# Tariq-Abuhashim/semantic-slam

Hardware: AMD Instinct MI355X
Metric: Mvoxels/sec integrated, 512³ grid @ 640×480 depth; achieved HBM GB/s %peak (higher is better)
Workload: dtype f32

## Files before the change

### include/tsdf_hip_diag.h

```cpp
#ifndef TSDF_HIP_DIAG_H
#define TSDF_HIP_DIAG_H

#include "tsdf_hip.h"

#ifdef __cplusplus
extern "C" {
#endif


int tsdf_integrate_sequence_timed(tsdf_volume *vol, const float *depth_dev, const float *cam2world,
                                  int32_t n_frames, float *elapsed_ms);

int tsdf_integrate_frames_timed(tsdf_volume *vol, const float *const *depth_dev, const uint8_t *const *masks_dev,
                                const float *cam2world, int32_t n_frames, float *elapsed_ms);


int tsdf_probe_graph_replay(tsdf_volume *vol, const float *depth_dev, const float *cam2world, int32_t n_frames,
                            int32_t iters, float *ms_launches, float *ms_graph);

int tsdf_probe_stream(tsdf_volume *vol, int32_t non_temporal, int32_t n_iters, float *elapsed_ms);


int tsdf_selftest_fastdiv(int32_t device, uint64_t seed, uint64_t n_samples, float fx, float cx,
                          uint64_t *mismatches, float first_bad[4]);

int tsdf_selftest_fastdiv_band(int32_t device, uint64_t seed, uint64_t n_samples, uint64_t *mismatches,
                               float first_bad[4]);

int tsdf_selftest_round(int32_t device, uint64_t *mismatches, float first_bad[4]);

int tsdf_selftest_tile_tables(int32_t device, const float *depth_dev, const uint8_t *mask_dev, int32_t im_height,
                              int32_t im_width, float max_depth, uint64_t *mismatches);


int32_t tsdf_frames_per_launch(const tsdf_volume *vol);
int tsdf_shortcut_stats(tsdf_volume *vol, int32_t enable, uint64_t counts_out[3]);
int tsdf_brick_list_stats(tsdf_volume *vol, uint64_t counts_out[4]);
int tsdf_classification_info(tsdf_volume *vol, double info_out[2]);

int tsdf_summary_stats(tsdf_volume *vol, uint64_t out[3]);
int tsdf_summary_words(tsdf_volume *vol, uint32_t *out_host, int64_t capacity, int64_t *count);

int tsdf_store_stats(tsdf_volume *vol, int64_t out[9]);

int tsdf_last_cam2base(const tsdf_volume *vol, float out[16]);


int tsdf_set_kernel_variant(tsdf_volume *vol, int32_t variant);

int tsdf_set_brick_shape(tsdf_volume *vol, int32_t quads, int32_t rows, int32_t slices);
int tsdf_brick_shape(const tsdf_volume *vol, int32_t shape_out[3]);
int tsdf_default_brick_shape(const tsdf_config *cfg, int32_t shape_out[3]);

#ifdef __cplusplus
}
#endif
#endif
```

### semantic_slam_amd/capi.py

```python
import ctypes as C
import os

import numpy as np

_PKG = os.path.dirname(os.path.abspath(__file__))
LIB_PATH = os.environ.get("TSDF_HIP_LIB") or os.path.join(_PKG, "libtsdf_hip.so")

ABI_SYMBOLS = [
    "tsdf_config_default", "tsdf_create", "tsdf_destroy", "tsdf_reset", "tsdf_integrate",
    "tsdf_integrate_u16", "tsdf_convert_depth_u16", "tsdf_set_deferral",
    "tsdf_integrate_device", "tsdf_integrate_cam2base", "tsdf_integrate_masked_device",
    "tsdf_integrate_frames_device",
    "tsdf_sync", "tsdf_download", "tsdf_copy_slices", "tsdf_upload", "tsdf_refresh_summary", "tsdf_device_ptrs", "tsdf_slab_voxels", "tsdf_frames_per_launch", "tsdf_shortcut_stats", "tsdf_brick_list_stats", "tsdf_classification_info", "tsdf_store_stats", "tsdf_summary_stats", "tsdf_summary_words",
    "tsdf_get_config", "tsdf_last_cam2base", "tsdf_set_stream", "tsdf_get_stream",
    "tsdf_count_surface", "tsdf_extract_surface", "tsdf_extract_crossings", "tsdf_extract_mesh", "tsdf_save_mesh_ply", "tsdf_save_mesh_welded_ply", "tsdf_save_ply", "tsdf_save_bin", "tsdf_load_bin", "tsdf_save_state", "tsdf_load_state",
    "tsdf_integrate_sequence_timed", "tsdf_integrate_frames_timed", "tsdf_probe_graph_replay", "tsdf_probe_stream", "tsdf_selftest_fastdiv", "tsdf_selftest_fastdiv_band", "tsdf_selftest_round", "tsdf_selftest_tile_tables", "tsdf_set_kernel_variant", "tsdf_set_brick_shape", "tsdf_brick_shape", "tsdf_default_brick_shape", "tsdf_last_error",
    "tsdf_version", "tsdf_multiply_matrix", "tsdf_invert_matrix",
    "tsdf_labels_enable", "tsdf_compose_labels", "tsdf_integrate_labels_device", "tsdf_integrate_frames_labels_device",
    "tsdf_download_labels",
    "tsdf_colour_enable", "tsdf_integrate_colour_device", "tsdf_integrate_rgbd", "tsdf_download_colour",
    "tsdf_raycast_params_default", "tsdf_raycast_device", "tsdf_raycast", "tsdf_batch_raycast_device",
    "tsdf_track_params_default", "tsdf_track", "tsdf_track_system",
    "tsdf_batch_track", "tsdf_batch_track_system", "tsdf_track_member_systems",
    "tsdf_fuse_params_default", "tsdf_fuse_volume",
    "tsdf_extent_params_default", "tsdf_volume_extent", "tsdf_batch_extents", "tsdf_group_extent", "tsdf_extent_combine",
    "tsdf_extent_metric", "tsdf_extent_regrid",
    "tsdf_associate_params_default", "tsdf_associate_count", "tsdf_associate_assign", "tsdf_batch_associate",
    "tsdf_segment_params_default", "tsdf_segmenter_create", "tsdf_segmenter_destroy", "tsdf_segmenter_set_stream",
    "tsdf_segment_depth_device", "tsdf_segment_refine_masks_device", "tsdf_segment_frame",
    "tsdf_object_origin", "tsdf_batch_create", "tsdf_batch_destroy", "tsdf_batch_size", "tsdf_batch_volume",
    "tsdf_batch_integrate_device", "tsdf_batch_sync",
    "tsdf_group_create", "tsdf_group_destroy", "tsdf_group_size", "tsdf_group_voxels", "tsdf_group_volume",
    "tsdf_group_integrate", "tsdf_group_integrate_frames", "tsdf_group_set_deferral", "tsdf_group_sync", "tsdf_group_reset", "tsdf_group_download",
    "tsdf_group_extract_surface", "tsdf_group_extract_crossings", "tsdf_group_extract_mesh",
    "tsdf_group_save_ply", "tsdf_group_save_mesh_ply", "tsdf_group_save_bin",
]
DIAG_SYMBOLS = [
    "tsdf_integrate_sequence_timed", "tsdf_integrate_frames_timed",
    "tsdf_probe_graph_replay", "tsdf_probe_stream",
    "tsdf_selftest_fastdiv", "tsdf_selftest_fastdiv_band", "tsdf_selftest_round", "tsdf_selftest_tile_tables",
    "tsdf_shortcut_stats", "tsdf_brick_list_stats", "tsdf_classification_info", "tsdf_store_stats", "tsdf_summary_stats", "tsdf_summary_words", "tsdf_frames_per_launch", "tsdf_last_cam2base",
    "tsdf_set_kernel_variant", "tsdf_set_brick_shape", "tsdf_brick_shape", "tsdf_default_brick_shape",
]


class TsdfError(RuntimeError):
    pass


SHIPPED_VARIANTS = (0, 1, 3, 7, 8)


def experiments_build():
    return b"+experiments" in load().tsdf_version()


def variants(*wanted):
    exp = experiments_build()
    return [v for v in wanted if v in SHIPPED_VARIANTS or exp]


class TsdfConfig(C.Structure):
    _fields_ = [
        ("im_height", C.c_int32), ("im_width", C.c_int32),
# ... 106 lines not shown
    L.tsdf_destroy.argtypes = [vp]
    L.tsdf_reset.argtypes = [vp]
    L.tsdf_integrate.argtypes = [vp, vp, vp]
    L.tsdf_set_deferral.argtypes = [vp, C.c_int32]
    L.tsdf_integrate_u16.argtypes = [vp, vp, C.c_float, C.c_int32, C.c_int32, vp]
    L.tsdf_convert_depth_u16.argtypes = [vp, vp, vp, C.c_float, C.c_int32, C.c_int32]
    L.tsdf_integrate_device.argtypes = [vp, vp, vp]
    L.tsdf_integrate_cam2base.argtypes = [vp, vp, vp]
    L.tsdf_integrate_masked_device.argtypes = [vp, vp, vp, vp]
    L.tsdf_integrate_frames_device.argtypes = [vp, vp, vp, vp, C.c_int32]
    L.tsdf_sync.argtypes = [vp]
    L.tsdf_download.argtypes = [vp, vp, vp]
    L.tsdf_upload.argtypes = [vp, vp, vp]
    L.tsdf_copy_slices.argtypes = [vp, C.c_int32, C.c_int32, vp, vp]
    L.tsdf_refresh_summary.argtypes = [vp]
    L.tsdf_device_ptrs.argtypes = [vp, C.POINTER(vp), C.POINTER(vp)]
    L.tsdf_slab_voxels.argtypes = [vp]
    L.tsdf_slab_voxels.restype = C.c_int64
    L.tsdf_frames_per_launch.argtypes = [vp]
    L.tsdf_frames_per_launch.restype = C.c_int32
    L.tsdf_shortcut_stats.argtypes = [vp, C.c_int32, vp]
    L.tsdf_classification_info.argtypes = [vp, vp]
    L.tsdf_brick_list_stats.argtypes = [vp, vp]
    if hasattr(L, "tsdf_store_stats"):
        L.tsdf_store_stats.argtypes = [vp, i64p]
    if hasattr(L, "tsdf_summary_stats"):
        L.tsdf_summary_stats.argtypes = [vp, vp]
    if hasattr(L, "tsdf_summary_words"):
        L.tsdf_summary_words.argtypes = [vp, vp, C.c_int64, i64p]
    L.tsdf_get_config.argtypes = [vp, C.POINTER(TsdfConfig)]
    L.tsdf_last_cam2base.argtypes = [vp, vp]
    L.tsdf_set_stream.argtypes = [vp, vp]
    L.tsdf_get_stream.argtypes = [vp, C.POINTER(vp)]
    L.tsdf_count_surface.argtypes = [vp, C.c_float, i64p]
    L.tsdf_extract_surface.argtypes = [vp, C.c_float, vp, C.c_int64, i64p]
    L.tsdf_extract_crossings.argtypes = [vp, vp, vp, C.c_float, vp, C.c_int64, i64p]
    L.tsdf_extract_mesh.argtypes = [vp, vp, vp, C.c_float, vp, C.c_int64, i64p]
    L.tsdf_save_mesh_ply.argtypes = [vp, C.c_char_p, C.c_float]
    L.tsdf_save_mesh_welded_ply.argtypes = [vp, C.c_char_p, C.c_float]
    L.tsdf_save_ply.argtypes = [vp, C.c_char_p, C.c_float]
    L.tsdf_save_bin.argtypes = [vp, C.c_char_p]
    L.tsdf_load_bin.argtypes = [vp, C.c_char_p]
    L.tsdf_save_state.argtypes = [vp, C.c_char_p]
    L.tsdf_load_state.argtypes = [vp, C.c_char_p]
    L.tsdf_integrate_sequence_timed.argtypes = [vp, vp, vp, C.c_int32, f32p]
    L.tsdf_integrate_frames_timed.argtypes = [vp, vp, vp, vp, C.c_int32, f32p]
    L.tsdf_probe_graph_replay.argtypes = [vp, vp, vp, C.c_int32, C.c_int32, f32p, f32p]
    L.tsdf_probe_stream.argtypes = [vp, C.c_int32, C.c_int32, f32p]
    L.tsdf_selftest_fastdiv.argtypes = [C.c_int32, C.c_uint64, C.c_uint64, C.c_float, C.c_float, C.POINTER(C.c_uint64), f32p]
    L.tsdf_selftest_fastdiv_band.argtypes = [C.c_int32, C.c_uint64, C.c_uint64, C.POINTER(C.c_uint64), f32p]
    L.tsdf_selftest_round.argtypes = [C.c_int32, C.POINTER(C.c_uint64), f32p]
    L.tsdf_selftest_tile_tables.argtypes = [C.c_int32, vp, vp, C.c_int32, C.c_int32, C.c_float, C.POINTER(C.c_uint64)]
    L.tsdf_set_kernel_variant.argtypes = [vp, C.c_int32]
    L.tsdf_set_brick_shape.argtypes = [vp, C.c_int32, C.c_int32, C.c_int32]
    L.tsdf_brick_shape.argtypes = [vp, C.POINTER(C.c_int32)]
    L.tsdf_default_brick_shape.argtypes = [C.POINTER(TsdfConfig), C.POINTER(C.c_int32)]
    L.tsdf_last_error.restype = C.c_char_p
    L.tsdf_version.restype = C.c_char_p
    L.tsdf_multiply_matrix.argtypes = [vp, vp, vp]
    L.tsdf_multiply_matrix.restype = None
    L.tsdf_invert_matrix.argtypes = [vp, vp]
    L.tsdf_labels_enable.argtypes = [vp, C.c_float]
    L.tsdf_compose_labels.argtypes = [vp, vp, vp, vp, C.c_int32, vp, vp]
    L.tsdf_integrate_labels_device.argtypes = [vp, vp, vp, vp, vp]
    L.tsdf_download_labels.argtypes = [vp, vp, vp, vp]
    L.tsdf_integrate_frames_labels_device.argtypes = [vp, vp, vp, vp, vp, C.c_int32]
    L.tsdf_colour_enable.argtypes = [vp]
    L.tsdf_integrate_colour_device.argtypes = [vp, vp, vp, vp]
    L.tsdf_integrate_rgbd.argtypes = [vp, vp, vp, vp]
    L.tsdf_download_colour.argtypes = [vp, vp]
    L.tsdf_raycast_params_default.argtypes = [C.POINTER(TsdfConfig), C.POINTER(RaycastParams)]
    L.tsdf_raycast_device.argtypes = [vp, C.POINTER(RaycastParams), vp, vp, vp, vp, vp]
    L.tsdf_raycast.argtypes = [vp, C.POINTER(RaycastParams), vp, vp, vp, vp, vp]
# ... 101 lines not shown


def invert_matrix(m):
    out = np.zeros(16, np.float32)
    m = _f32(m, 16)
    ok = load().tsdf_invert_matrix(m.ctypes.data, out.ctypes.data)
    return bool(ok), out


def selftest_fastdiv(n_samples, seed=1, device=0, fx=535.4, cx=320.1):
    cnt = C.c_uint64()
    bad = (C.c_float * 4)()
    check(load().tsdf_selftest_fastdiv(device, seed, n_samples, fx, cx, C.byref(cnt), bad), "tsdf_selftest_fastdiv")
    return cnt.value, list(bad)


def selftest_fastdiv_band(n_samples, seed=1, device=0):
    cnt = C.c_uint64()
    bad = (C.c_float * 4)()
    check(load().tsdf_selftest_fastdiv_band(device, seed, n_samples, C.byref(cnt), bad), "tsdf_selftest_fastdiv_band")
    return cnt.value, list(bad)


def object_origin(depth_ptr, mask_ptr, h, w, K, device=0):
    k = _f32(K, 9)
    out = np.empty(3, np.float32)
    check(load().tsdf_object_origin(device, depth_ptr, mask_ptr, h, w, k.ctypes.data, out.ctypes.data), "tsdf_object_origin")
    return out


def raycast_params_default(cfg):
    p = RaycastParams()
    check(load().tsdf_raycast_params_default(C.byref(cfg), C.byref(p)), "tsdf_raycast_params_default")
    return p


def track_params_default(cfg):
    p = TrackParams()
    check(load().tsdf_track_params_default(C.byref(cfg), C.byref(p)), "tsdf_track_params_default")
    return p


def fuse_params_default(cfg):
    p = FuseParams()
    check(load().tsdf_fuse_params_default(C.byref(cfg), C.byref(p)), "tsdf_fuse_params_default")
    return p
# ... 172 lines not shown
        return self

    def __exit__(self, *exc):
        self.close()

    def __del__(self):
        try:
            self.close()
        except Exception:
            pass

    @property
    def n_voxels(self):
        return int(self.lib.tsdf_slab_voxels(self._h))

    def shortcut_stats(self, enable=True):
        out = (C.c_uint64 * 3)()
        check(self.lib.tsdf_shortcut_stats(self._h, 1 if enable else 0, out), "tsdf_shortcut_stats")
        return tuple(int(x) for x in out)

    def brick_list_stats(self):
        out = (C.c_uint64 * 4)()
        check(self.lib.tsdf_brick_list_stats(self._h, out), "tsdf_brick_list_stats")
        return tuple(int(x) for x in out)

    def classification_info(self):
        out = (C.c_double * 2)()
        check(self.lib.tsdf_classification_info(self._h, out), "tsdf_classification_info")
        return float(out[0]), int(out[1])

    def store_stats(self):
        out = (C.c_int64 * 9)()
        check(self.lib.tsdf_store_stats(self._h, out), "tsdf_store_stats")
        return {name: tuple(int(x) for x in out[3 * k:3 * k + 3]) for k, name in enumerate(("frames", "masks", "tables"))}

    def summary_stats(self):
        out = (C.c_uint64 * 3)()
        check(self.lib.tsdf_summary_stats(self._h, out), "tsdf_summary_stats")
        return tuple(int(x) for x in out)

    def summary_words(self):
        n = C.c_int64(0)
        check(self.lib.tsdf_summary_words(self._h, None, 0, C.byref(n)), "tsdf_summary_words")
        out = np.zeros(int(n.value), np.uint32)
        if out.size:
            check(self.lib.tsdf_summary_words(self._h, out.ctypes.data, out.size, C.byref(n)), "tsdf_summary_words")
# ... 516 lines not shown
```

### semantic_slam_amd/csrc/tsdf_diag.hip.h

```cpp
#pragma once

namespace {

template <typename Queue>
int time_on_stream(tsdf_volume *v, const char *who, float *elapsed_ms, Queue &&queue)
{
    Event e0, e1;
    HIP_TRY(event_create(e0, hipEventDefault));
    HIP_TRY(event_create(e1, hipEventDefault));
    HIP_TRY(hipEventRecord(e0, v->stream));
    const int rc = queue();
    hipError_t er = hipEventRecord(e1, v->stream);
    hipError_t es = hipEventSynchronize(e1);
    float ms = 0.f;
    hipError_t et = hipEventElapsedTime(&ms, e0, e1);
    if (rc) return rc;
    if (er != hipSuccess || es != hipSuccess || et != hipSuccess)
        return fail(TSDF_ERR_HIP, "%s: event timing failed", who);
    *elapsed_ms = ms;
    return TSDF_OK;
}

int frames_timed(tsdf_volume *v, const float *const *depth_dev, const uint8_t *const *masks_dev,
                 const float *cam2world, int32_t n_frames, float *elapsed_ms, const char *who)
// ... 108 lines not shown
    if (e == hipSuccess) e = hipMemcpy(first_bad, d_bad, 4 * sizeof(float), hipMemcpyDeviceToHost);
    if (e != hipSuccess) return fail(TSDF_ERR_HIP, "tsdf_selftest_fastdiv: %s", hipGetErrorString(e));
    *mismatches = cnt;
    return TSDF_OK;
}

int tsdf_selftest_fastdiv_band(int32_t device, uint64_t seed, uint64_t n_samples, uint64_t *mismatches, float first_bad[4])
{
    if (!mismatches || !first_bad) return fail(TSDF_ERR_INVALID, "tsdf_selftest_fastdiv_band: NULL argument");
    HIP_TRY(hipSetDevice(device));
    DevPtr<unsigned long long> d_cnt;
    DevPtr<float> d_bad;
    HIP_TRY(dev_alloc(d_cnt, sizeof(unsigned long long)));
    HIP_TRY(dev_alloc(d_bad, 4 * sizeof(float)));
    HIP_TRY(hipMemset(d_cnt, 0, sizeof(unsigned long long)));
    HIP_TRY(hipMemset(d_bad, 0, 4 * sizeof(float)));
    hipLaunchKernelGGL(tsdfk::selftest_fastdiv_band, dim3(256 * 8), dim3(256), 0, 0, seed, n_samples, d_cnt, d_bad);
    hipError_t e = hipGetLastError();
    if (e == hipSuccess) e = hipDeviceSynchronize();
    unsigned long long cnt = 0;
    if (e == hipSuccess) e = hipMemcpy(&cnt, d_cnt, sizeof cnt, hipMemcpyDeviceToHost);
    if (e == hipSuccess) e = hipMemcpy(first_bad, d_bad, 4 * sizeof(float), hipMemcpyDeviceToHost);
    if (e != hipSuccess) return fail(TSDF_ERR_HIP, "tsdf_selftest_fastdiv_band: %s", hipGetErrorString(e));
    *mismatches = cnt;
    return TSDF_OK;
}

int tsdf_selftest_round(int32_t device, uint64_t *mismatches, float first_bad[4])
{
    if (!mismatches || !first_bad) return fail(TSDF_ERR_INVALID, "tsdf_selftest_round: NULL argument");
    HIP_TRY(hipSetDevice(device));
    DevPtr<unsigned long long> d_cnt;
    DevPtr<float> d_bad;
    HIP_TRY(dev_alloc(d_cnt, sizeof(unsigned long long)));
    HIP_TRY(dev_alloc(d_bad, 4 * sizeof(float)));
    HIP_TRY(hipMemset(d_cnt, 0, sizeof(unsigned long long)));
    HIP_TRY(hipMemset(d_bad, 0, 4 * sizeof(float)));
    hipLaunchKernelGGL(tsdfk::selftest_round, dim3(256 * 8), dim3(256), 0, 0, d_cnt, d_bad);
    hipError_t e = hipGetLastError();
    if (e == hipSuccess) e = hipDeviceSynchronize();
    unsigned long long cnt = 0;
    if (e == hipSuccess) e = hipMemcpy(&cnt, d_cnt, sizeof cnt, hipMemcpyDeviceToHost);
    if (e == hipSuccess) e = hipMemcpy(first_bad, d_bad, 4 * sizeof(float), hipMemcpyDeviceToHost);
    if (e != hipSuccess) return fail(TSDF_ERR_HIP, "tsdf_selftest_round: %s", hipGetErrorString(e));
    *mismatches = cnt;
    return TSDF_OK;
// ... 90 lines not shown
    }
    *mismatches = bad;
    return TSDF_OK;
}


int32_t tsdf_frames_per_launch(const tsdf_volume *v)
{
    if (!v) return 0;
    return can_fuse(v) ? frames_per_launch(v) : 1;
}

int tsdf_shortcut_stats(tsdf_volume *v, int32_t enable, uint64_t counts_out[3])
{
    if (!v) return fail(TSDF_ERR_INVALID, "tsdf_shortcut_stats: NULL handle");
    int rc = bind_device(v);
    if (rc) return rc;
    HIP_TRY(hipStreamSynchronize(v->stream));
    if (counts_out) {
        unsigned int h[3] = {0, 0, 0};
        if (v->d_shortcut_stats) HIP_TRY(hipMemcpy(h, v->d_shortcut_stats, sizeof h, hipMemcpyDeviceToHost));
        for (int i = 0; i < 3; ++i) counts_out[i] = h[i];
    }
    if (enable && !v->d_shortcut_stats) HIP_TRY(dev_alloc(v->d_shortcut_stats, 8 * sizeof(unsigned int)));
    if (v->d_shortcut_stats) {
        if (enable) HIP_TRY(hipMemset(v->d_shortcut_stats, 0, 8 * sizeof(unsigned int)));
        else v->d_shortcut_stats.reset();
    }
    return TSDF_OK;
}

int tsdf_brick_list_stats(tsdf_volume *v, uint64_t counts_out[4])
{
    if (!v || !counts_out) return fail(TSDF_ERR_INVALID, "tsdf_brick_list_stats: NULL argument");
    int rc = bind_device(v);
    if (rc) return rc;
    HIP_TRY(hipStreamSynchronize(v->stream));
    unsigned int h[8] = {0, 0, 0, 0, 0, 0, 0, 0};
    if (v->d_shortcut_stats) HIP_TRY(hipMemcpy(h, v->d_shortcut_stats, sizeof h, hipMemcpyDeviceToHost));
    for (int i = 0; i < 4; ++i) counts_out[i] = h[3 + i];
    return TSDF_OK;
}

int tsdf_classification_info(tsdf_volume *v, double info_out[2])
{
    if (!v || !info_out) return fail(TSDF_ERR_INVALID, "tsdf_classification_info: NULL argument");
    int rc = bind_device(v);
    if (rc) return rc;
    HIP_TRY(hipStreamSynchronize(v->stream));
    if (v->rb_stream) HIP_TRY(hipStreamSynchronize(v->rb_stream));
    if (v->claims_pending && hipEventQuery(v->claims_done) == hipSuccess) {
        v->claim_fraction = claims_read_back(v);
        v->claims_pending = false;
        v->claims_known = true;
    }
    info_out[0] = v->claims_known ? v->claim_fraction : -1.0;
    info_out[1] = (double)v->launches_unclassified;
    return TSDF_OK;
}

int tsdf_summary_stats(tsdf_volume *v, uint64_t out[3])
{
    if (!v || !out) return fail(TSDF_ERR_INVALID, "tsdf_summary_stats: NULL argument");
// ... 85 lines not shown
```

### semantic_slam_amd/csrc/tsdf_kernels.hip.h

```cpp
#pragma once
#include <hip/hip_runtime.h>
#include <stdint.h>
#include <type_traits>

#include "host_derive.h"

namespace tsdfk {

struct IntegrateParams {
    const float *depth;
    const uint8_t *mask;
    float *tsdf;
    float *weight;
    float fx, fy, cx, cy;
    float rx0, rx1, rx2;
    float ry0, ry1, ry2;
    float rz0, rz1, rz2;
    float tx, ty, tz;
    float ox, oy, oz;
    float vs, trunc, max_depth;
    int dim_x, dim_y;
    int nz, z_begin;
    int H, W;
    int xgroups;
    uint32_t *flags;
    int nseg;
    int quads_per_row, quads_per_slice, chunks_per_slice;
    int brick_q, brick_r, brick_s, bricks_per_group, brick_groups;
    int brick_q_magic, brick_per_magic;
    int fast_ok;
// ... 450 lines not shown
        const uint32_t mode = h2 & 7u;
        uint32_t dm = h0 & 0x7fffffu;
        if (mode == 1) dm = 0x7fffffu; else if (mode == 2) dm = 0u; else if (mode == 3) dm &= 0x7u;
        const uint32_t de = 127u - 20u + (h0 >> 23) % 41u;
        const float d = __uint_as_float((de << 23) | dm);
        uint32_t ne = 127u - 81u + (h1 >> 23) % 142u;
        if (mode >= 6) ne = de - 2u + (h1 >> 23) % 5u;
        if (ne > 127u + 60u) ne = 127u + 60u;
        uint32_t nm = h1 & 0x7fffffu;
        if (mode == 4) nm = 0x7fffffu; else if (mode == 5) nm = dm;
        if (ne == 127u + 60u) nm = 0u;
        float n = __uint_as_float((((h2 >> 3) & 1u) << 31) | (ne << 23) | nm);
        if (((h2 >> 5) & 63u) == 0u) n = 0.0f;
        if (((h2 >> 5) & 63u) == 1u) n = __uint_as_float(0x7fc00000u | (h2 >> 12));
        const float q = fast_div_r(n, d, refined_rcp(d));
        const float r = n / d;
        const bool same = __float_as_uint(q) == __float_as_uint(r) || (q != q && r != r);
        if (!same) {
            if (atomicAdd(mismatch, 1ull) == 0ull) { first_bad[0] = n; first_bad[1] = d; first_bad[2] = q; first_bad[3] = r; }
        }
    }
}

__global__ __launch_bounds__(256) void selftest_round(unsigned long long *mismatch, float *first_bad)
{
    const uint64_t stride = (uint64_t)gridDim.x * blockDim.x;
    const uint64_t n_pos = 0x4B800001ull, n_neg = 0x3F000000ull;
    for (uint64_t i = (uint64_t)blockIdx.x * blockDim.x + threadIdx.x; i < n_pos + n_neg; i += stride) {
        const uint32_t bits = i < n_pos ? (uint32_t)i : (0x80000000u + (uint32_t)(i - n_pos));
        const float u = __uint_as_float(bits);
        if (!(u > -0.5f)) continue;
        const int want = (int)roundf(u);
        const int got = round_half_up_i32(u);
        if (got != want) {
            if (atomicAdd(mismatch, 1ull) == 0ull) { first_bad[0] = u; first_bad[1] = (float)got; first_bad[2] = (float)want; first_bad[3] = 0.f; }
        }
    }
}

template <bool NT>
__global__ __launch_bounds__(256) void stream_rmw(float *tsdf, float *weight, size_t n_quads, float one,
                                                  float zero)
{
    const size_t stride = (size_t)gridDim.x * blockDim.x;
    for (size_t q = (size_t)blockIdx.x * blockDim.x + threadIdx.x; q < n_quads; q += stride) {
        float4 t = vol_load<NT>(tsdf + 4 * q);
// ... 112 lines not shown
```

### semantic_slam_amd/csrc/tsdf_multiframe.hip.h

```cpp
#pragma once
#include "launch_geometry.h"
#include "tsdf_kernels.hip.h"

namespace tsdfk {

constexpr int kMaxFramesPerLaunch = 32;
constexpr int kFineTile = 4;
constexpr int kFineLevels = 3;
__host__ __device__ inline size_t fine_table_elems(int fw, int fh) { return (size_t)kFineLevels * kFineLevels * fw * fh; }

struct FramePose {
    const float *depth;
    const uint8_t *mask;
    float rx0, ry0, rx1, ry1, rx2, ry2, rz0, rz1, rz2, tz, tx, ty;
    int fast_ok;
    float cz_margin;
    const uint16_t *label_im;
    const float *score_im;
    const float2 *tiles;
    float cz_short;
    float cz_pad;
};

constexpr int kListBuckets = 64;
// ... 517 lines not shown
    cls[id] = (uint8_t)c;
}

struct LabelState {
    uint16_t *label;
    float *fp, *bp;
    float prob_thd;
};

struct MultiParamsInline {
    IntegrateParams common;
    FramePose frames[kMaxFramesPerLaunch];
    int n_frames;
    LabelState labels;
    int z_fastest;
#ifdef TSDF_EXPERIMENTS
    const unsigned int *super_mask;
    int nz_super;
#endif
};

constexpr int kSuperZ = 4;

template <int R, bool NT, bool FLAT, bool LABELS = false, bool MASKS = true, bool SHORT = false, bool BRICK = false, bool EAGER_W = false>
__device__ __forceinline__ void multi_body(const IntegrateParams &p, const FramePose *__restrict__ frames,
                                           const int n_frames, const int b0, const int b1, const int lz,
                                           const LabelState ls = LabelState(), const unsigned int free_frames = 0u,
                                           const unsigned int skip_frames = 0u)
{
    static_assert(!SHORT || R == 1, "patch classification is written for one row per lane");
    static_assert(!LABELS || R == 1, "label fusion rides on the one-row kernel");
    static_assert(!FLAT || R == 1, "the flat mapping handles one quad per lane");
    static_assert(!BRICK || (R == 1 && !FLAT), "bricks are their own mapping");
    static_assert(!EAGER_W || BRICK, "eager weights are for the bricks of a work list");
    int xg, gy0;
    size_t row0, flag0;
    size_t brick_base = 0;
    unsigned int lane_byte = 0u;
    uint32_t flag32 = 0u;
    constexpr bool kBuf = BRICK && !NT;
    __amdgpu_buffer_rsrc_t t_buf, w_buf;
    auto load_quad = [&](const bool tsdf, const int r) -> float4 {
        if constexpr (kBuf) {
            const v4u v = __builtin_amdgcn_raw_buffer_load_b128(tsdf ? t_buf : w_buf, (int)lane_byte, 0, 0);
            return make_float4(__uint_as_float(v.x), __uint_as_float(v.y), __uint_as_float(v.z), __uint_as_float(v.w));
        } else {
            return vol_load<NT>((tsdf ? p.tsdf : p.weight) + row0 + (size_t)r * p.dim_x);
        }
    };
    auto store_quad = [&](const bool tsdf, const int r, const float4 q) {
        if constexpr (kBuf) {
            const v4u v = {__float_as_uint(q.x), __float_as_uint(q.y), __float_as_uint(q.z), __float_as_uint(q.w)};
            __builtin_amdgcn_raw_buffer_store_b128(v, tsdf ? t_buf : w_buf, (int)lane_byte, 0, 0);
        } else {
            vol_store<NT>((tsdf ? p.tsdf : p.weight) + row0 + (size_t)r * p.dim_x, q);
        }
    };
// ... 25 lines not shown
        const int chunk = b0 * 4 + threadIdx.y;
        const int q = chunk * 64 + threadIdx.x;
        if (q >= p.quads_per_slice) return;
        gy0 = q / p.quads_per_row;
        xg = q - gy0 * p.quads_per_row;
        row0 = ((size_t)lz * p.quads_per_slice + q) * 4;
        flag0 = (size_t)lz * p.chunks_per_slice + chunk;
    } else {
        xg = b0 * 64 + threadIdx.x;
        gy0 = (b1 * 4 + threadIdx.y) * R;
        if (xg >= p.xgroups || gy0 >= p.dim_y) return;
        row0 = ((size_t)lz * p.dim_y + gy0) * (size_t)p.dim_x + (size_t)xg * 4;
        flag0 = ((size_t)lz * p.dim_y + gy0) * (size_t)p.nseg + b0;
    }
    const int gz = p.z_begin + lzz;

    uint32_t fl[R];
    bool ones[R];
    float4 t4[R], w4[R];
    bool touched[R], tchanged[R];
#pragma unroll
    for (int r = 0; r < R; ++r) {
        fl[r] = (R == 1 || gy0 + r < p.dim_y) ? p.flags[flag0 + (size_t)r * p.nseg] : 0u;
        ones[r] = (fl[r] & 1u) != 0u;
        t4[r] = make_float4(1.f, 1.f, 1.f, 1.f);
        w4[r] = make_float4(0.f, 0.f, 0.f, 0.f);
        touched[r] = tchanged[r] = false;
    }
    bool have_w = false;
    if constexpr (EAGER_W) {
        w4[0] = load_quad(false, 0);
        have_w = true;
    }

    float bxv[4], byv[R];
#pragma unroll
    for (int j = 0; j < 4; ++j) bxv[j] = p.ox + (float)(xg * 4 + j) * p.vs;
#pragma unroll
    for (int r = 0; r < R; ++r) byv[r] = p.oy + (float)(gy0 + r) * p.vs;
    const float bz = p.oz + (float)gz * p.vs;
    const v2f F = {p.fx, p.fy}, C = {p.cx, p.cy};
    const float trunc_r1 = refined_rcp(p.trunc);
    bool fast_frame = false;

    float diff[R][4];
    bool upd[R][4], rowany[R], bandr[R];
    bool any = false, band = false;
    auto apply_frame = [&]() __attribute__((always_inline)) {
#pragma unroll
        for (int r = 0; r < R; ++r) {
            if (rowany[r] && !touched[r]) {
                if (!have_w) w4[r] = load_quad(false, r);
                if (!(fl[r] & 1u)) t4[r] = load_quad(true, r);
                touched[r] = true;
            }
        }
        float dist[R][4];
        if (__ballot(band) != 0ull) {
            if (fast_frame && p.trunc_fast != 0) {
#pragma unroll
                for (int r = 0; r < R; ++r)
#pragma unroll
                    for (int j = 0; j < 4; ++j) dist[r][j] = fminf(1.0f, fast_div_r(diff[r][j], p.trunc, trunc_r1));
            } else {
#pragma unroll
                for (int r = 0; r < R; ++r)
#pragma unroll
                    for (int j = 0; j < 4; ++j) dist[r][j] = fminf(1.0f, diff[r][j] / p.trunc);
            }
        } else {
#pragma unroll
            for (int r = 0; r < R; ++r)
#pragma unroll
                for (int j = 0; j < 4; ++j) dist[r][j] = 1.0f;
        }

#pragma unroll
        for (int r = 0; r < R; ++r) {
            if (__ballot(!(ones[r] && (fl[r] & 2u)) || bandr[r]) == 0ull) {
                if (upd[r][0]) w4[r].x += 1.0f;
                if (upd[r][1]) w4[r].y += 1.0f;
                if (upd[r][2]) w4[r].z += 1.0f;
                if (upd[r][3]) w4[r].w += 1.0f;
                continue;
            }
            float tv[4] = {t4[r].x, t4[r].y, t4[r].z, t4[r].w};
            float wv[4] = {w4[r].x, w4[r].y, w4[r].z, w4[r].w};
            float num[4], wn[4];
            const bool wave_band = __ballot(bandr[r]) != 0ull;
            bool need = false;
#pragma unroll
            for (int j = 0; j < 4; ++j) {
                wn[j] = wv[j] + 1.0f;
                num[j] = tv[j] * wv[j] + dist[r][j];
            }
            if (!wave_band) {
#pragma unroll
                for (int j = 0; j < 4; ++j) need |= upd[r][j] && !(num[j] == wn[j] && wn[j] < 3.0e38f && wn[j] > 0.0f);
// ... 44 lines not shown
                    touched[0] = true;
                    const unsigned int rest = ~(free_frames >> f);
                    unsigned int run = rest != 0u ? (unsigned)(__ffs((int)rest) - 1) : 32u - (unsigned)f;
                    run = min(run, (unsigned)(n_frames - f));
                    const float4 w = w4[0];
                    const bool whole = w.x == truncf(w.x) && w.y == truncf(w.y) && w.z == truncf(w.z) && w.w == truncf(w.w) &&
                                       fmaxf(fmaxf(w.x, w.y), fmaxf(w.z, w.w)) < 16777184.0f;
                    if (run > 1u && __ballot(!whole) == 0ull) {
                        const float k = (float)run;
                        w4[0].x += k; w4[0].y += k; w4[0].z += k; w4[0].w += k;
                        todo &= ~((run >= 32u ? 0xffffffffu : ((1u << run) - 1u)) << f);
                        if (p.shortcut_stats != nullptr && (threadIdx.x & 63) == 0) atomicAdd(p.shortcut_stats + 1, run);
                        continue;
                    }
                    if (p.shortcut_stats != nullptr && (threadIdx.x & 63) == 0) atomicAdd(p.shortcut_stats + 1, 1u);
                    w4[0].x += 1.0f; w4[0].y += 1.0f; w4[0].z += 1.0f; w4[0].w += 1.0f;
                    continue;
                }
                if (p.shortcut_stats != nullptr && (threadIdx.x & 63) == 0) atomicAdd(p.shortcut_stats + 1, 1u);
#pragma unroll
                for (int r = 0; r < R; ++r) {
                    rowany[r] = true;
                    bandr[r] = false;
#pragma unroll
                    for (int j = 0; j < 4; ++j) { upd[r][j] = true; diff[r][j] = p.trunc; }
                }
                band = false;
                apply_frame();
                continue;
            }
        }
        if constexpr (SHORT) {
            if (p.shortcut_stats != nullptr && (threadIdx.x & 63) == 0) atomicAdd(p.shortcut_stats, 1u);
        }
        any = false;
        band = false;
        {
        const FramePose q = frames[f];

        float ax[4], ay[4], az[4];
#pragma unroll
        for (int j = 0; j < 4; ++j) {
            const float dx = bxv[j] - q.tx;
            ax[j] = q.rx0 * dx; ay[j] = q.ry0 * dx; az[j] = q.rz0 * dx;
        }
        const float dz = bz - q.tz;
// ... 59 lines not shown
                    const float cz = pcz[r][j];
                    const float pu = roundf(p.fx * (cx / cz) + p.cx);
                    const float pv = roundf(p.fy * (cy / cz) + p.cy);
                    const bool ok = row_ok && !(cz <= 0.0f) && pu >= 0.0f && pu < (float)p.W && pv >= 0.0f &&
                                    pv < (float)p.H;
                    fetch(r, j, ok, ok ? (uint32_t)((int)pv * p.W + (int)pu) : 0u);
                }
            }
        }

        if constexpr (MASKS) {
            if (q.mask != nullptr) {
#pragma unroll
                for (int r = 0; r < R; ++r)
#pragma unroll
                    for (int j = 0; j < 4; ++j) dval[r][j] = dval[r][j] * (mval[r][j] >= 128 ? 1.0f : 0.0f);
            }
        }

#pragma unroll
        for (int r = 0; r < R; ++r) {
            rowany[r] = false;
            bandr[r] = false;
#pragma unroll
            for (int j = 0; j < 4; ++j) {
                const float d = dval[r][j];
                const float df = d - pcz[r][j];
                diff[r][j] = df;
                const bool u = !((d <= 0.0f) | (d > p.max_depth)) & !(df <= -p.trunc);
                upd[r][j] = u;
                rowany[r] |= u;
                bandr[r] |= u & !(df >= p.trunc);
            }
            band |= bandr[r];
            any |= rowany[r];
        }
        if (__ballot(any) == 0ull) continue;

        if constexpr (LABELS) {
            if (q.label_im != nullptr && __ballot(band) != 0ull) {
                uint16_t lab_in[4];
                float sc_in[4];
                bool hit = false;
#pragma unroll
                for (int j = 0; j < 4; ++j) {
                    const bool seen = upd[0][j] & (diff[0][j] < p.trunc);
                    lab_in[j] = 0;
                    sc_in[j] = 0.0f;
                    if (seen) { lab_in[j] = q.label_im[pixel[0][j]]; sc_in[j] = q.score_im[pixel[0][j]]; }
                    hit |= lab_in[j] != 0;
                }
                if (hit) {
                    ushort4 L4 = *reinterpret_cast<const ushort4 *>(ls.label + row0);
                    float4 F4 = *reinterpret_cast<const float4 *>(ls.fp + row0);
// ... 25 lines not shown
        apply_frame();
    }

#pragma unroll
    for (int r = 0; r < R; ++r) {
        const bool store_t = __ballot(touched[r] && tchanged[r]) != 0ull;
        if (touched[r]) {
            if (store_t) store_quad(true, r, t4[r]);
            store_quad(false, r, w4[r]);
        }
        if ((fl[r] & 1u) && !ones[r]) {
            if constexpr (BRICK) {
                p.flags[flag32] = fl[r] & 2u;
            } else {
                p.flags[flag0 + (size_t)r * p.nseg] = fl[r] & 2u;
            }
        }
    }
}

#ifndef TSDF_BRICK_WAVES
#define TSDF_BRICK_WAVES 8
#endif
template <int R, bool NT, bool FLAT, bool LABELS = false, bool MASKS = true>
__global__ __launch_bounds__(256, R == 2 ? 6 : 1) void integrate_multi_inline(MultiParamsInline mp)
{
    typedef const char __attribute__((address_space(4))) *kernarg_ptr;
    kernarg_ptr base = (kernarg_ptr)__builtin_amdgcn_kernarg_segment_ptr();
    typedef const FramePose __attribute__((address_space(4))) *frames_ptr;
    frames_ptr frames = (frames_ptr)(base + offsetof(MultiParamsInline, frames));
    const int wg_x = mp.z_fastest ? (int)blockIdx.z : (int)blockIdx.x, wg_y = (int)blockIdx.y;
    int wg_z = mp.z_fastest ? (int)blockIdx.x : (int)blockIdx.z;
    if (mp.z_fastest == 2) {
        wg_z += (int)((unsigned)(wg_x + wg_y) % gridDim.x);
        if (wg_z >= (int)gridDim.x) wg_z -= (int)gridDim.x;
    }
    multi_body<R, NT, FLAT, LABELS, MASKS>(mp.common, (const FramePose *)frames, mp.n_frames, wg_x, wg_y, wg_z, mp.labels);
}

constexpr int kSuperBX = 4, kSuperBY = 2, kSuperBZ = 1;
constexpr int kSuperBricks = kSuperBX * kSuperBY * kSuperBZ;
static_assert(kSuperBricks <= 32, "one lane of a half-wave per brick of the super-brick");
constexpr unsigned int kBrickUndecided = 0x80000000u;

struct BrickListParams {
    uint4 *list;
    unsigned char *counters;
    unsigned int bucket_cap;
    ClassPoseTable *poses;
    int nsx, nsy, nsz;
    int wedge_mode, wedge_oy, wedge_oz, super_h, super_d, fy_px;
};


__global__ __launch_bounds__(256) void classify_brick_list(MultiParamsInline mp, BrickListParams bl)
{
    typedef const char __attribute__((address_space(4))) *kernarg_ptr;
    kernarg_ptr base = (kernarg_ptr)__builtin_amdgcn_kernarg_segment_ptr();
    const FramePose *frames = (const FramePose *)(base + offsetof(MultiParamsInline, frames));
    const IntegrateParams &p = mp.common;
// ... 76 lines not shown
        const int lane = threadIdx.x;
        const unsigned int frames_mask = mp.n_frames >= 32 ? 0xffffffffu : ((1u << mp.n_frames) - 1u);
        const int g = brick / p.bricks_per_group, i = brick - g * p.bricks_per_group;
        const int xa = i * p.brick_q * 4, ya = g * p.brick_r;
        const int z0 = zg * p.brick_s, z1 = min(z0 + p.brick_s - 1, p.nz - 1);
        const float2 *fine_f = p.fine != nullptr ? p.fine + (size_t)(lane & 31) * fine_table_elems(p.fine_w, p.fine_h) : nullptr;
        const int cls = classify_patch<true>(p, class_pose(poses, lane & 31), xa, xa + p.brick_q * 4 - 1, ya, min(ya + p.brick_r - 1, p.dim_y - 1),
                                             p.z_begin + z0, p.z_begin + z1, fine_f);
        free_frames |= (unsigned int)__ballot(cls == 1) & frames_mask;
        skip_frames |= (unsigned int)__ballot(cls == 2) & frames_mask;
        free_frames = __builtin_amdgcn_readfirstlane(free_frames);
        skip_frames = __builtin_amdgcn_readfirstlane(skip_frames);
        if (skip_frames == frames_mask) {
            if (p.shortcut_stats != nullptr && lane == 0) { atomicAdd(p.shortcut_stats + 2, (unsigned)mp.n_frames); atomicAdd(p.shortcut_stats + 6, 1u); }
            return;
        }
    }
    multi_body<1, NT, false, LABELS, MASKS, true, true, true>(mp.common, frames, mp.n_frames, brick, 0, zg, mp.labels, free_frames, skip_frames);
}

template <bool NT, bool FLAT>
__global__ __launch_bounds__(256) void integrate_multi_single(IntegrateParams p, FramePose pose)
{
    multi_body<1, NT, FLAT>(p, &pose, 1, blockIdx.x, blockIdx.y, blockIdx.z);
}

template <bool NT>
__global__ __launch_bounds__(256) void integrate_multi_batched(const IntegrateParams *__restrict__ params,
                                                               const FramePose *__restrict__ poses,
                                                               const int2 *__restrict__ slice_map)
{
    const int2 m = slice_map[blockIdx.z];
    const IntegrateParams p = params[m.x];
    multi_body<1, NT, true>(p, poses + m.x, 1, blockIdx.x, 0, m.y);
}

template <bool NT>
__global__ __launch_bounds__(256, 8) void integrate_single_bricks(IntegrateParams p, FramePose pose)
{
    const unsigned c = p.wg_class[(blockIdx.x + gridDim.x * blockIdx.z) * 4u + threadIdx.y];
    if (c == 2u) return;
    multi_body<1, NT, false, false, true, true, true>(p, &pose, 1, (int)blockIdx.x * 4 + __builtin_amdgcn_readfirstlane((int)threadIdx.y), 0,
                                                      blockIdx.z, LabelState(), c == 1u ? 1u : 0u, 0u);
}

template <bool NT>
__global__ __launch_bounds__(256, 8) void integrate_multi_batched_bricks(const IntegrateParams *__restrict__ params,
// ... 34 lines not shown
```

Before: 500,800.

## Add wave-uniform count mode that replaces weighted averaging with running-count division

Adds a COUNT template path to the multi-frame integrator. When a wave's voxel weights are all the same integer, it tracks a scalar count instead of per-voxel weights. Frames that leave a free-space row at ones skip the distance computation, and other frames use a fast exact division by count+1 with a fallback to true division. It also adds a bit-exactness selftest for the divide and counters for the guarded and fallback paths. The aim is less per-voxel arithmetic and weight handling in the R==1 paths, at the cost of extra ballots, readfirstlane calls and code size.

Result: no change. 503,800 (median of 5 runs) (+0.6%).

```diff
diff --git a/include/tsdf_hip_diag.h b/include/tsdf_hip_diag.h
--- a/include/tsdf_hip_diag.h
+++ b/include/tsdf_hip_diag.h
@@ -27,6 +27,9 @@
 int tsdf_selftest_fastdiv_band(int32_t device, uint64_t seed, uint64_t n_samples, uint64_t *mismatches,
                                float first_bad[4]);
 
+int tsdf_selftest_fastdiv_count(int32_t device, uint64_t seed, uint64_t n_samples, uint64_t *mismatches,
+                                float first_bad[4]);
+
 int tsdf_selftest_round(int32_t device, uint64_t *mismatches, float first_bad[4]);
 
 int tsdf_selftest_tile_tables(int32_t device, const float *depth_dev, const uint8_t *mask_dev, int32_t im_height,
@@ -36,6 +39,7 @@
 int32_t tsdf_frames_per_launch(const tsdf_volume *vol);
 int tsdf_shortcut_stats(tsdf_volume *vol, int32_t enable, uint64_t counts_out[3]);
 int tsdf_brick_list_stats(tsdf_volume *vol, uint64_t counts_out[4]);
+int tsdf_count_mode_stats(tsdf_volume *vol, uint64_t counts_out[2]);
 int tsdf_classification_info(tsdf_volume *vol, double info_out[2]);
 
 int tsdf_summary_stats(tsdf_volume *vol, uint64_t out[3]);
diff --git a/semantic_slam_amd/capi.py b/semantic_slam_amd/capi.py
--- a/semantic_slam_amd/capi.py
+++ b/semantic_slam_amd/capi.py
@@ -11,10 +11,10 @@
     "tsdf_integrate_u16", "tsdf_convert_depth_u16", "tsdf_set_deferral",
     "tsdf_integrate_device", "tsdf_integrate_cam2base", "tsdf_integrate_masked_device",
     "tsdf_integrate_frames_device",
-    "tsdf_sync", "tsdf_download", "tsdf_copy_slices", "tsdf_upload", "tsdf_refresh_summary", "tsdf_device_ptrs", "tsdf_slab_voxels", "tsdf_frames_per_launch", "tsdf_shortcut_stats", "tsdf_brick_list_stats", "tsdf_classification_info", "tsdf_store_stats", "tsdf_summary_stats", "tsdf_summary_words",
+    "tsdf_sync", "tsdf_download", "tsdf_copy_slices", "tsdf_upload", "tsdf_refresh_summary", "tsdf_device_ptrs", "tsdf_slab_voxels", "tsdf_frames_per_launch", "tsdf_shortcut_stats", "tsdf_brick_list_stats", "tsdf_count_mode_stats", "tsdf_classification_info", "tsdf_store_stats", "tsdf_summary_stats", "tsdf_summary_words",
     "tsdf_get_config", "tsdf_last_cam2base", "tsdf_set_stream", "tsdf_get_stream",
     "tsdf_count_surface", "tsdf_extract_surface", "tsdf_extract_crossings", "tsdf_extract_mesh", "tsdf_save_mesh_ply", "tsdf_save_mesh_welded_ply", "tsdf_save_ply", "tsdf_save_bin", "tsdf_load_bin", "tsdf_save_state", "tsdf_load_state",
-    "tsdf_integrate_sequence_timed", "tsdf_integrate_frames_timed", "tsdf_probe_graph_replay", "tsdf_probe_stream", "tsdf_selftest_fastdiv", "tsdf_selftest_fastdiv_band", "tsdf_selftest_round", "tsdf_selftest_tile_tables", "tsdf_set_kernel_variant", "tsdf_set_brick_shape", "tsdf_brick_shape", "tsdf_default_brick_shape", "tsdf_last_error",
+    "tsdf_integrate_sequence_timed", "tsdf_integrate_frames_timed", "tsdf_probe_graph_replay", "tsdf_probe_stream", "tsdf_selftest_fastdiv", "tsdf_selftest_fastdiv_band", "tsdf_selftest_fastdiv_count", "tsdf_selftest_round", "tsdf_selftest_tile_tables", "tsdf_set_kernel_variant", "tsdf_set_brick_shape", "tsdf_brick_shape", "tsdf_default_brick_shape", "tsdf_last_error",
     "tsdf_version", "tsdf_multiply_matrix", "tsdf_invert_matrix",
     "tsdf_labels_enable", "tsdf_compose_labels", "tsdf_integrate_labels_device", "tsdf_integrate_frames_labels_device",
     "tsdf_download_labels",
@@ -38,8 +38,8 @@
 DIAG_SYMBOLS = [
     "tsdf_integrate_sequence_timed", "tsdf_integrate_frames_timed",
     "tsdf_probe_graph_replay", "tsdf_probe_stream",
-    "tsdf_selftest_fastdiv", "tsdf_selftest_fastdiv_band", "tsdf_selftest_round", "tsdf_selftest_tile_tables",
-    "tsdf_shortcut_stats", "tsdf_brick_list_stats", "tsdf_classification_info", "tsdf_store_stats", "tsdf_summary_stats", "tsdf_summary_words", "tsdf_frames_per_launch", "tsdf_last_cam2base",
+    "tsdf_selftest_fastdiv", "tsdf_selftest_fastdiv_band", "tsdf_selftest_fastdiv_count", "tsdf_selftest_round", "tsdf_selftest_tile_tables",
+    "tsdf_shortcut_stats", "tsdf_brick_list_stats", "tsdf_count_mode_stats", "tsdf_classification_info", "tsdf_store_stats", "tsdf_summary_stats", "tsdf_summary_words", "tsdf_frames_per_launch", "tsdf_last_cam2base",
     "tsdf_set_kernel_variant", "tsdf_set_brick_shape", "tsdf_brick_shape", "tsdf_default_brick_shape",
 ]
 
@@ -192,6 +192,8 @@
     L.tsdf_shortcut_stats.argtypes = [vp, C.c_int32, vp]
     L.tsdf_classification_info.argtypes = [vp, vp]
     L.tsdf_brick_list_stats.argtypes = [vp, vp]
+    if hasattr(L, "tsdf_count_mode_stats"):
+        L.tsdf_count_mode_stats.argtypes = [vp, vp]
     if hasattr(L, "tsdf_store_stats"):
         L.tsdf_store_stats.argtypes = [vp, i64p]
     if hasattr(L, "tsdf_summary_stats"):
@@ -219,6 +221,8 @@
     L.tsdf_probe_stream.argtypes = [vp, C.c_int32, C.c_int32, f32p]
     L.tsdf_selftest_fastdiv.argtypes = [C.c_int32, C.c_uint64, C.c_uint64, C.c_float, C.c_float, C.POINTER(C.c_uint64), f32p]
     L.tsdf_selftest_fastdiv_band.argtypes = [C.c_int32, C.c_uint64, C.c_uint64, C.POINTER(C.c_uint64), f32p]
+    if hasattr(L, "tsdf_selftest_fastdiv_count"):
+        L.tsdf_selftest_fastdiv_count.argtypes = [C.c_int32, C.c_uint64, C.c_uint64, C.POINTER(C.c_uint64), f32p]
     L.tsdf_selftest_round.argtypes = [C.c_int32, C.POINTER(C.c_uint64), f32p]
     L.tsdf_selftest_tile_tables.argtypes = [C.c_int32, vp, vp, C.c_int32, C.c_int32, C.c_float, C.POINTER(C.c_uint64)]
     L.tsdf_set_kernel_variant.argtypes = [vp, C.c_int32]
@@ -366,6 +370,13 @@
     return cnt.value, list(bad)
 
 
+def selftest_fastdiv_count(n_samples, seed=1, device=0):
+    cnt = C.c_uint64()
+    bad = (C.c_float * 4)()
+    check(load().tsdf_selftest_fastdiv_count(device, seed, n_samples, C.byref(cnt), bad), "tsdf_selftest_fastdiv_count")
+    return cnt.value, list(bad)
+
+
 def object_origin(depth_ptr, mask_ptr, h, w, K, device=0):
     k = _f32(K, 9)
     out = np.empty(3, np.float32)
@@ -584,6 +595,11 @@
     def brick_list_stats(self):
         out = (C.c_uint64 * 4)()
         check(self.lib.tsdf_brick_list_stats(self._h, out), "tsdf_brick_list_stats")
+        return tuple(int(x) for x in out)
+
+    def count_mode_stats(self):
+        out = (C.c_uint64 * 2)()
+        check(self.lib.tsdf_count_mode_stats(self._h, out), "tsdf_count_mode_stats")
         return tuple(int(x) for x in out)
 
     def classification_info(self):
diff --git a/semantic_slam_amd/csrc/tsdf_diag.hip.h b/semantic_slam_amd/csrc/tsdf_diag.hip.h
--- a/semantic_slam_amd/csrc/tsdf_diag.hip.h
+++ b/semantic_slam_amd/csrc/tsdf_diag.hip.h
@@ -154,6 +154,27 @@
     if (e == hipSuccess) e = hipMemcpy(&cnt, d_cnt, sizeof cnt, hipMemcpyDeviceToHost);
     if (e == hipSuccess) e = hipMemcpy(first_bad, d_bad, 4 * sizeof(float), hipMemcpyDeviceToHost);
     if (e != hipSuccess) return fail(TSDF_ERR_HIP, "tsdf_selftest_fastdiv_band: %s", hipGetErrorString(e));
+    *mismatches = cnt;
+    return TSDF_OK;
+}
+
+int tsdf_selftest_fastdiv_count(int32_t device, uint64_t seed, uint64_t n_samples, uint64_t *mismatches, float first_bad[4])
+{
+    if (!mismatches || !first_bad) return fail(TSDF_ERR_INVALID, "tsdf_selftest_fastdiv_count: NULL argument");
+    HIP_TRY(hipSetDevice(device));
+    DevPtr<unsigned long long> d_cnt;
+    DevPtr<float> d_bad;
+    HIP_TRY(dev_alloc(d_cnt, sizeof(unsigned long long)));
+    HIP_TRY(dev_alloc(d_bad, 4 * sizeof(float)));
+    HIP_TRY(hipMemset(d_cnt, 0, sizeof(unsigned long long)));
+    HIP_TRY(hipMemset(d_bad, 0, 4 * sizeof(float)));
+    hipLaunchKernelGGL(tsdfk::selftest_fastdiv_count, dim3(256 * 8), dim3(256), 0, 0, seed, n_samples, d_cnt, d_bad);
+    hipError_t e = hipGetLastError();
+    if (e == hipSuccess) e = hipDeviceSynchronize();
+    unsigned long long cnt = 0;
+    if (e == hipSuccess) e = hipMemcpy(&cnt, d_cnt, sizeof cnt, hipMemcpyDeviceToHost);
+    if (e == hipSuccess) e = hipMemcpy(first_bad, d_bad, 4 * sizeof(float), hipMemcpyDeviceToHost);
+    if (e != hipSuccess) return fail(TSDF_ERR_HIP, "tsdf_selftest_fastdiv_count: %s", hipGetErrorString(e));
     *mismatches = cnt;
     return TSDF_OK;
 }
@@ -290,9 +311,9 @@
         if (v->d_shortcut_stats) HIP_TRY(hipMemcpy(h, v->d_shortcut_stats, sizeof h, hipMemcpyDeviceToHost));
         for (int i = 0; i < 3; ++i) counts_out[i] = h[i];
     }
-    if (enable && !v->d_shortcut_stats) HIP_TRY(dev_alloc(v->d_shortcut_stats, 8 * sizeof(unsigned int)));
+    if (enable && !v->d_shortcut_stats) HIP_TRY(dev_alloc(v->d_shortcut_stats, tsdfk::kShortcutStatWords * sizeof(unsigned int)));
     if (v->d_shortcut_stats) {
-        if (enable) HIP_TRY(hipMemset(v->d_shortcut_stats, 0, 8 * sizeof(unsigned int)));
+        if (enable) HIP_TRY(hipMemset(v->d_shortcut_stats, 0, tsdfk::kShortcutStatWords * sizeof(unsigned int)));
         else v->d_shortcut_stats.reset();
     }
     return TSDF_OK;
@@ -307,6 +328,18 @@
     unsigned int h[8] = {0, 0, 0, 0, 0, 0, 0, 0};
     if (v->d_shortcut_stats) HIP_TRY(hipMemcpy(h, v->d_shortcut_stats, sizeof h, hipMemcpyDeviceToHost));
     for (int i = 0; i < 4; ++i) counts_out[i] = h[3 + i];
+    return TSDF_OK;
+}
+
+int tsdf_count_mode_stats(tsdf_volume *v, uint64_t counts_out[2])
+{
+    if (!v || !counts_out) return fail(TSDF_ERR_INVALID, "tsdf_count_mode_stats: NULL argument");
+    int rc = bind_device(v);
+    if (rc) return rc;
+    HIP_TRY(hipStreamSynchronize(v->stream));
+    unsigned int h[tsdfk::kShortcutStatWords] = {};
+    if (v->d_shortcut_stats) HIP_TRY(hipMemcpy(h, v->d_shortcut_stats, sizeof h, hipMemcpyDeviceToHost));
+    for (int i = 0; i < 2; ++i) counts_out[i] = h[8 + i];
     return TSDF_OK;
 }
 
diff --git a/semantic_slam_amd/csrc/tsdf_kernels.hip.h b/semantic_slam_amd/csrc/tsdf_kernels.hip.h
--- a/semantic_slam_amd/csrc/tsdf_kernels.hip.h
+++ b/semantic_slam_amd/csrc/tsdf_kernels.hip.h
@@ -6,6 +6,8 @@
 #include "host_derive.h"
 
 namespace tsdfk {
+
+constexpr int kShortcutStatWords = 10;
 
 struct IntegrateParams {
     const float *depth;
@@ -502,6 +504,53 @@
     }
 }
 
+__global__ __launch_bounds__(256) void selftest_fastdiv_count(uint64_t seed, uint64_t n_samples, unsigned long long *mismatch,
+                                                              float *first_bad)
+{
+    const uint64_t stride = (uint64_t)gridDim.x * blockDim.x;
+    for (uint64_t i = (uint64_t)blockIdx.x * blockDim.x + threadIdx.x; i < (1ull << 24); i += stride) {
+        const float c = (float)(uint32_t)i, d = (float)((uint32_t)i + 1u);
+        const float r1 = refined_rcp(d);
+        auto check = [&](const float n) {
+            const float a = fabsf(n);
+            if (!((a >= 0x1p-60f) & (a < 0x1p25f))) return;
+            const float q = fast_div_r(n, d, r1);
+            const float r = n / d;
+            if (__float_as_uint(q) != __float_as_uint(r)) {
+                if (atomicAdd(mismatch, 1ull) == 0ull) { first_bad[0] = n; first_bad[1] = d; first_bad[2] = q; first_bad[3] = r; }
+            }
+        };
+        const uint32_t db = __float_as_uint(d);
+        const uint32_t fixed[10] = {0x21800000u, 0x21800001u, 0x4BFFFFFFu, 0x4BFFFFFEu, 0x4B800000u, db, db - 1u, db + 1u,
+                                    __float_as_uint(c), 0x3F800000u};
+#pragma unroll
+        for (int k = 0; k < 10; ++k) {
+            check(__uint_as_float(fixed[k]));
+            check(__uint_as_float(fixed[k] | 0x80000000u));
+        }
+        for (uint64_t k = 0; k < n_samples; ++k) {
+            const uint64_t at = seed + 2 * (i * n_samples + k);
+            const uint32_t h0 = hash32(at), h1 = hash32(at + 1);
+            const uint32_t mode = h1 & 7u, sign = (h1 >> 3) & 1u;
+            float n;
+            if (mode < 5u) {
+                uint32_t nm = h0 & 0x7fffffu;
+                if (mode == 2u) nm = 0x7fffffu; else if (mode == 3u) nm = 0u; else if (mode == 4u) nm &= 0x7u;
+                const uint32_t ne = 127u - 60u + (h0 >> 23) % 85u;
+                n = __uint_as_float((sign << 31) | (ne << 23) | nm);
+            } else {
+                float t = (float)(h0 & 0xffffffu) * 0x1p-24f;
+                if (mode == 7u) t = 1.0f;
+                if (sign) t = -t;
+                float dist = (float)(h1 >> 8) * 0x1p-23f - 1.0f;
+                if (mode == 6u) dist = 1.0f;
+                n = t * c + dist;
+            }
+            check(n);
+        }
+    }
+}
+
 __global__ __launch_bounds__(256) void selftest_round(unsigned long long *mismatch, float *first_bad)
 {
     const uint64_t stride = (uint64_t)gridDim.x * blockDim.x;
diff --git a/semantic_slam_amd/csrc/tsdf_multiframe.hip.h b/semantic_slam_amd/csrc/tsdf_multiframe.hip.h
--- a/semantic_slam_amd/csrc/tsdf_multiframe.hip.h
+++ b/semantic_slam_amd/csrc/tsdf_multiframe.hip.h
@@ -563,7 +563,8 @@
 
 constexpr int kSuperZ = 4;
 
-template <int R, bool NT, bool FLAT, bool LABELS = false, bool MASKS = true, bool SHORT = false, bool BRICK = false, bool EAGER_W = false>
+template <int R, bool NT, bool FLAT, bool LABELS = false, bool MASKS = true, bool SHORT = false, bool BRICK = false, bool EAGER_W = false,
+          bool COUNT = false>
 __device__ __forceinline__ void multi_body(const IntegrateParams &p, const FramePose *__restrict__ frames,
                                            const int n_frames, const int b0, const int b1, const int lz,
                                            const LabelState ls = LabelState(), const unsigned int free_frames = 0u,
@@ -574,6 +575,7 @@
     static_assert(!FLAT || R == 1, "the flat mapping handles one quad per lane");
     static_assert(!BRICK || (R == 1 && !FLAT), "bricks are their own mapping");
     static_assert(!EAGER_W || BRICK, "eager weights are for the bricks of a work list");
+    static_assert(!COUNT || (R == 1 && !BRICK && !SHORT), "count mode needs the row's ones flag wave-uniform and one row per lane");
     int xg, gy0;
     size_t row0, flag0;
     size_t brick_base = 0;
@@ -645,6 +647,7 @@
 #pragma unroll
     for (int r = 0; r < R; ++r) {
         fl[r] = (R == 1 || gy0 + r < p.dim_y) ? p.flags[flag0 + (size_t)r * p.nseg] : 0u;
+        if constexpr (COUNT) fl[r] = (uint32_t)__builtin_amdgcn_readfirstlane((int)fl[r]);
         ones[r] = (fl[r] & 1u) != 0u;
         t4[r] = make_float4(1.f, 1.f, 1.f, 1.f);
         w4[r] = make_float4(0.f, 0.f, 0.f, 0.f);
@@ -655,6 +658,8 @@
         w4[0] = load_quad(false, 0);
         have_w = true;
     }
+    bool cmode = false, ctried = false;
+    unsigned int cnt = 0u;
 
     float bxv[4], byv[R];
 #pragma unroll
@@ -668,6 +673,7 @@
 
     float diff[R][4];
     bool upd[R][4], rowany[R], bandr[R];
+    bool rowall[R];
     bool any = false, band = false;
     auto apply_frame = [&]() __attribute__((always_inline)) {
 #pragma unroll
@@ -678,7 +684,22 @@
                 touched[r] = true;
             }
         }
+        if constexpr (COUNT) {
+            if (!ctried) {
+                ctried = true;
+                const uint32_t wb = (uint32_t)__builtin_amdgcn_readfirstlane((int)__float_as_uint(w4[0].x));
+                const uint32_t bx = __float_as_uint(w4[0].x), by = __float_as_uint(w4[0].y), bz2 = __float_as_uint(w4[0].z),
+                               bw = __float_as_uint(w4[0].w);
+                const bool same = touched[0] & (bx == wb) & (by == wb) & (bz2 == wb) & (bw == wb);
+                const float wf = __uint_as_float(wb);
+                if (__ballot(!same) == 0ull && wb < 0x4B800000u && wf == truncf(wf)) {
+                    cmode = true;
+                    cnt = (unsigned int)__builtin_amdgcn_readfirstlane((int)(unsigned int)wf);
+                }
+            }
+        }
         float dist[R][4];
+        auto truncated_distance = [&]() __attribute__((always_inline)) {
         if (__ballot(band) != 0ull) {
             if (fast_frame && p.trunc_fast != 0) {
 #pragma unroll
@@ -697,6 +718,58 @@
 #pragma unroll
                 for (int j = 0; j < 4; ++j) dist[r][j] = 1.0f;
         }
+        };
+
+        if constexpr (COUNT) {
+            if (cmode) {
+                if (__ballot(!rowall[0]) == 0ull && cnt < (1u << 24)) {
+                    const bool wave_band = __ballot(bandr[0]) != 0ull;
+                    const bool wave_ones = __ballot(ones[0]) != 0ull;
+                    w4[0].x += 1.0f; w4[0].y += 1.0f; w4[0].z += 1.0f; w4[0].w += 1.0f;
+                    if (wave_ones && !wave_band) {
+                        cnt += 1u;
+                        return;
+                    }
+                    truncated_distance();
+                    const float cf = (float)cnt, c1 = (float)(cnt + 1u);
+                    const float tv[4] = {t4[0].x, t4[0].y, t4[0].z, t4[0].w};
+                    float num[4], nt[4];
+#pragma unroll
+                    for (int j = 0; j < 4; ++j) num[j] = tv[j] * cf + dist[0][j];
+                    const float amax = fmaxf(fmaxf(fabsf(num[0]), fabsf(num[1])), fmaxf(fabsf(num[2]), fabsf(num[3])));
+                    const float amin = fminf(fminf(fabsf(num[0]), fabsf(num[1])), fminf(fabsf(num[2]), fabsf(num[3])));
+                    const bool inside = (amin >= 0x1p-60f) & (amax < 0x1p25f) &
+                                        !__builtin_isunordered(num[0], num[1]) & !__builtin_isunordered(num[2], num[3]);
+                    const bool guarded = __ballot(!inside) == 0ull;
+                    if (guarded) {
+                        const float r1 = refined_rcp(c1);
+#pragma unroll
+                        for (int j = 0; j < 4; ++j) nt[j] = fast_div_r(num[j], c1, r1);
+                    } else {
+#pragma unroll
+                        for (int j = 0; j < 4; ++j) nt[j] = num[j] / c1;
+                    }
+                    if (p.shortcut_stats != nullptr && (threadIdx.x & 63) == 0) atomicAdd(p.shortcut_stats + (guarded ? 8 : 9), 1u);
+                    bool changed = wave_band;
+                    if (!wave_band) {
+#pragma unroll
+                        for (int j = 0; j < 4; ++j) changed |= __float_as_uint(nt[j]) != __float_as_uint(tv[j]);
+                    }
+                    if (wave_ones) {
+                        bool notone = false;
+#pragma unroll
+                        for (int j = 0; j < 4; ++j) notone |= __float_as_uint(nt[j]) != 0x3f800000u;
+                        if (__ballot(notone) != 0ull) ones[0] = false;
+                    }
+                    t4[0] = make_float4(nt[0], nt[1], nt[2], nt[3]);
+                    tchanged[0] |= changed;
+                    cnt += 1u;
+                    return;
+                }
+                cmode = false;
+            }
+        }
+        truncated_distance();
 
 #pragma unroll
         for (int r = 0; r < R; ++r) {
@@ -787,6 +860,7 @@
                 for (int r = 0; r < R; ++r) {
                     rowany[r] = true;
                     bandr[r] = false;
+                    rowall[r] = true;
 #pragma unroll
                     for (int j = 0; j < 4; ++j) { upd[r][j] = true; diff[r][j] = p.trunc; }
                 }
@@ -892,6 +966,7 @@
         for (int r = 0; r < R; ++r) {
             rowany[r] = false;
             bandr[r] = false;
+            rowall[r] = true;
 #pragma unroll
             for (int j = 0; j < 4; ++j) {
                 const float d = dval[r][j];
@@ -900,6 +975,7 @@
                 const bool u = !((d <= 0.0f) | (d > p.max_depth)) & !(df <= -p.trunc);
                 upd[r][j] = u;
                 rowany[r] |= u;
+                rowall[r] &= u;
                 bandr[r] |= u & !(df >= p.trunc);
             }
             band |= bandr[r];
@@ -971,6 +1047,7 @@
 #ifndef TSDF_BRICK_WAVES
 #define TSDF_BRICK_WAVES 8
 #endif
+constexpr bool count_mode_in(int R, bool FLAT, bool LABELS, bool MASKS) { return R == 1; }
 template <int R, bool NT, bool FLAT, bool LABELS = false, bool MASKS = true>
 __global__ __launch_bounds__(256, R == 2 ? 6 : 1) void integrate_multi_inline(MultiParamsInline mp)
 {
@@ -984,7 +1061,8 @@
         wg_z += (int)((unsigned)(wg_x + wg_y) % gridDim.x);
         if (wg_z >= (int)gridDim.x) wg_z -= (int)gridDim.x;
     }
-    multi_body<R, NT, FLAT, LABELS, MASKS>(mp.common, (const FramePose *)frames, mp.n_frames, wg_x, wg_y, wg_z, mp.labels);
+    multi_body<R, NT, FLAT, LABELS, MASKS, false, false, false, count_mode_in(R, FLAT, LABELS, MASKS)>(
+        mp.common, (const FramePose *)frames, mp.n_frames, wg_x, wg_y, wg_z, mp.labels);
 }
 
 constexpr int kSuperBX = 4, kSuperBY = 2, kSuperBZ = 1;
@@ -1107,7 +1185,7 @@
 template <bool NT, bool FLAT>
 __global__ __launch_bounds__(256) void integrate_multi_single(IntegrateParams p, FramePose pose)
 {
-    multi_body<1, NT, FLAT>(p, &pose, 1, blockIdx.x, blockIdx.y, blockIdx.z);
+    multi_body<1, NT, FLAT, false, true, false, false, false, count_mode_in(1, FLAT, false, true)>(p, &pose, 1, blockIdx.x, blockIdx.y, blockIdx.z);
 }
 
 template <bool NT>
```
